# lzyhha/VisualCloze

Hardware: AMD Instinct MI355X
Metric: denoising-steps/sec (higher is better)
Workload: dtype bf16; 1 GPU; 384-grid-2x3 in-context, 30 solver points = 29 Flux evaluations per grid, L=512+3456 tokens, FLUX.1-Fill-dev geometry + LoRA r256 (merged), random-init weights, 1 independent grid(s) per GPU (data-parallel, no in-step collective); global_batch=1, seq_len=3968, parallelism=dp1

## Files before the change

### visualcloze_amd/csrc/attention64.hip

```cpp
#include <type_traits>
#include "common.h"
#include "vcloze_internal.h"
#include "attention64_sched8.h"

using namespace vcplan;

namespace {

struct Attn64Args {
  const bf16_t* qkv;
  const bf16_t* vt;
  bf16_t* out;
  const int32_t* kv_len;
  const int32_t* kv_gap;
  int64_t ld, bstride, ldo, out_bstride;
  int32_t B, L, Lpad, H, qblocks, items;
  int32_t full_rounds, tail_items, tail_units;
  float* part;
  const bf16_t* q_scale; const bf16_t* q_scale2; const float* rope; int64_t rope_bstride; int32_t split;
  int32_t q_pre;
  int32_t inmerge;
  uint32_t* flags;
  uint64_t* debug_ts;
};

constexpr int V_RING0 = RING * K_TILE;

constexpr int A_O = 0, A_Q = 128, A_K = 192;

typedef _Float16 f16x4 __attribute__((ext_vector_type(4)));
VC_DEV int chunk_begin64(int c, int units, int chunks) { return (int)(((long)c * units) / chunks); }
VC_DEV void merge_fold64(float (&acc)[16][4], float& wsum, float& m, const f16x4 (&v)[16], const f32x2 ml) {
  const float m_new = fmaxf(m, ml[0]);
  const float keep = __builtin_amdgcn_exp2f(m - m_new);
  const float w = ml[1] * __builtin_amdgcn_exp2f(ml[0] - m_new);
  m = m_new;
  wsum = __builtin_fmaf(wsum, keep, w);
#pragma unroll
  for (int i = 0; i < 16; ++i)
#pragma unroll
    for (int e = 0; e < 4; ++e) acc[i][e] = __builtin_fmaf(w, (float)v[i][e], acc[i][e] * keep);
}

VC_DEV int swap23(int i) { return (i & ~12) | ((i & 4) << 1) | ((i & 8) >> 1); }

template <int I, int N, class F>
VC_DEV void sfor(F&& f) {
  if constexpr (I < N) {
    f(std::integral_constant<int, I>{});
    sfor<I + 1, N>(f);
  }
}
#define SB() __builtin_amdgcn_sched_barrier(0)
template <int PH, int I>
constexpr a64s::Tok tok_at() {
  if constexpr (PH == 0) return a64s::A_TOK[I];
  else return a64s::B_TOK[I];
}

template <int KA, int QA, bool ZERO>
VC_DEV void mfma_qk(f32x16& s) {
  if constexpr (ZERO)
    asm volatile("v_mfma_f32_32x32x16_bf16 %0, a[%c1:%c2], a[%c3:%c4], 0" : "=v"(s) : "n"(KA), "n"(KA + 3), "n"(QA), "n"(QA + 3));
  else
    asm volatile("v_mfma_f32_32x32x16_bf16 %0, a[%c1:%c2], a[%c3:%c4], %0" : "+v"(s) : "n"(KA), "n"(KA + 3), "n"(QA), "n"(QA + 3));
}
VC_DEV void mfma_aug(f32x16& s, const u32x4& k, const u32x4& q) {
  asm volatile("v_mfma_f32_32x32x16_bf16 %0, %1, %2, %0" : "+v"(s) : "v"(k), "v"(q));
}
template <int OA>
VC_DEV void mfma_pv(const u32x4& v, const u32x4& p) {
  asm volatile("v_mfma_f32_32x32x16_bf16 a[%c2:%c3], %0, %1, a[%c2:%c3]" ::"v"(v), "v"(p), "n"(OA), "n"(OA + 15));
}
template <int A0, int OFF>
VC_DEV void lds_k(uint32_t addr) {
  asm volatile("ds_read_b128 a[%c1:%c2], %0 offset:%c3" ::"v"(addr), "n"(A0), "n"(A0 + 3), "n"(OFF));
}
template <int OFF>
VC_DEV void lds_v(u32x4& f, uint32_t addr) {
  asm volatile("ds_read_b128 %0, %1 offset:%c2" : "=v"(f) : "v"(addr), "n"(OFF));
}
template <int A0, int OFF>
VC_DEV void load_q(const bf16_t* p) {
  asm volatile("global_load_dwordx4 a[%c1:%c2], %0, off offset:%c3" ::"v"(p), "n"(A0), "n"(A0 + 3), "n"(OFF) : "memory");
}
template <int N> VC_DEV void wait_lgkm() { asm volatile("s_waitcnt lgkmcnt(%c0)" ::"n"(N)); }
template <int N> VC_DEV void wait_vm() { asm volatile("s_waitcnt vmcnt(%c0)" ::"n"(N)); }
VC_DEV float v_max3(float a, float b, float c) {
  float r;
  asm("v_max3_f32 %0, %1, %2, %3" : "=v"(r) : "v"(a), "v"(b), "v"(c));
  return r;
}
VC_DEV float v_max(float a, float b) {
  float r;
  asm("v_max_f32 %0, %1, %2" : "=v"(r) : "v"(a), "v"(b));
  return r;
}
#define PIN(x) asm volatile("" : "+v"(x))
VC_DEV uint32_t v_cvt_pk(float lo, float hi) {
  uint32_t r;
  asm("v_cvt_pk_bf16_f32 %0, %1, %2" : "=v"(r) : "v"(lo), "v"(hi));
  return r;
}
#pragma clang diagnostic push
#pragma clang diagnostic ignored "-Winline-asm"
VC_DEV void glds16_m0(const char* sbase, uint32_t voff, uint32_t lds_wave, int imm) {
  asm volatile("s_add_u32 m0, %2, %3\n\ts_nop 0\n\tglobal_load_lds_dwordx4 %0, %1" ::"v"(voff), "s"(sbase), "s"(lds_wave), "i"(imm) : "memory", "m0", "scc");
}
#pragma clang diagnostic pop
template <int A> VC_DEV float agpr_read() {
  float r;
  asm volatile("v_accvgpr_read_b32 %0, a[%c1]" : "=v"(r) : "n"(A));
  return r;
}
template <int A> VC_DEV void agpr_write(float v) { asm volatile("v_accvgpr_write_b32 a[%c1], %0" ::"v"(v), "n"(A)); }
VC_DEV void half_swap(float x, float& lo, float& hi) {
  asm volatile("v_mov_b32 %1, %2\n\tv_mov_b32 %0, %2\n\ts_nop 1\n\tv_permlane32_swap_b32 %0, %1" : "=&v"(lo), "=&v"(hi) : "v"(x));
}
VC_DEV float xmax32(float x) {
  float lo, hi;
  half_swap(x, lo, hi);
  return v_max(lo, hi);
}
VC_DEV float xsum32(float x) {
  float lo, hi;
  half_swap(x, lo, hi);
  return lo + hi;
}

template <bool BOUNDED>
__global__ __launch_bounds__(256, 1) void attn64_kernel(const Attn64Args a) {
  extern __shared__ __attribute__((aligned(16))) char smem[];
  asm volatile("" ::: "a0", "a15", "a31", "a47", "a63", "a79", "a95", "a111", "a127", "a143", "a159", "a175", "a191", "a207",
               "a223", "a239", "a255");

  const int tid = threadIdx.x;
  const int lane = tid & 63;
  const int wave = __builtin_amdgcn_readfirstlane(tid >> 6);
  const int lq = lane & 31, hh = lane >> 5;
  const float c_scale = 0.08838834764831845f * 1.4426950408889634f;
  const float MASKED = -29952.0f;

  uint32_t k_rd[8], v_rd[4];
  const int krow = swap23(lq);
  {
#pragma unroll
    for (int t = 0; t < 8; ++t) k_rd[t] = krow * 256 + (((2 * t + hh) ^ (krow & 15)) << 4);
#pragma unroll
    for (int s = 0; s < 4; ++s) v_rd[s] = V_RING0 + lq * 128 + (((2 * s + hh) ^ ((lq >> 1) & 7)) << 4);
  }
  uint32_t k_off[4], v_off[4];
#pragma unroll
  for (int i = 0; i < 4; ++i) {
    const int c = i * 256 + tid;
    const int row = c >> 4;
    k_off[i] = (uint32_t)row * (uint32_t)a.ld * 2u + (uint32_t)(((c & 15) ^ (row & 15)) << 4);
    const int d = c >> 3;
    v_off[i] = ((uint32_t)d * (uint32_t)a.Lpad + (uint32_t)((((c & 7) ^ ((d >> 1) & 7))) << 3)) * 2u;
  }
  const uint32_t k_step = (uint32_t)KVB * (uint32_t)a.ld * 2u;
  const uint32_t k_max = (uint32_t)(a.L - 1) * (uint32_t)a.ld * 2u + (uint32_t)(((tid & 15) ^ ((tid >> 4) & 15)) << 4);
  const uint32_t aug_on = hh == 0 ? 0xffffffffu : 0u;
  const uint32_t kaug_one = 0x3f80u & aug_on;
  const uint32_t qaug_mask = ((uint32_t)f2bf(MASKED) << 16) & aug_on;

#ifdef VC_ATTN_TIMESTAMPS
  const uint64_t ts0 = __builtin_amdgcn_s_memtime();
  int ts_tiles = 0, ts_seg = 0;
#define TS_SEG(k) do { if (a.debug_ts && tid == 0 && ts_seg < 3) a.debug_ts[blockIdx.x * 32 + 8 + ts_seg * 8 + (k)] = __builtin_amdgcn_s_memtime(); } while (0)
#else
#define TS_SEG(k) do { } while (0)
#endif
  const int G = gridDim.x;
  const int nkt_all = (a.L + KVB - 1) / KVB;
  const bool split = a.full_rounds >= 0;
  int tu = 0, tu_end = 0, it_first = 0, rounds_left = 0x7fffffff, id_full = blockIdx.x, id_step = G, id_tail = 0;
  if (split) {
    const int slot = blockIdx.x >> 3;
    const Sched64 sc = sched64(blockIdx.x & 7, G, a.items, nkt_all);
    tu = chunk_begin64(slot, sc.units, sc.W);
    tu_end = chunk_begin64(slot + 1, sc.units, sc.W);
    it_first = tu / nkt_all;
    rounds_left = sc.rounds;
    id_full = sc.start + slot;
    id_step = sc.W;
    id_tail = sc.start + sc.rounds * sc.W;
  }

  for (;;) {
    int id, kt0 = 0, kt1 = -1, piece = -1;
    if (rounds_left > 0) {
      if (!split && id_full >= a.items) break;
      id = split ? id_full : xcd_remap(id_full, a.items);
      id_full += id_step;
      --rounds_left;
    } else {
      if (tu >= tu_end) break;
      const int it = tu / nkt_all;
      kt0 = tu - it * nkt_all;
      kt1 = min(nkt_all, kt0 + (tu_end - tu));
      tu += kt1 - kt0;
      id = id_tail + it;
      if (kt1 - kt0 != nkt_all) piece = blockIdx.x * 2 + (it - it_first);
    }
    const int qb_i = id % a.qblocks;
    const int bh = id / a.qblocks;
    const int h = bh % a.H, b = bh / a.H;
    const int L = a.L;
    const int kvlen = a.kv_len ? __builtin_amdgcn_readfirstlane(a.kv_len[b]) : L;
    const int gap_lo = a.kv_gap ? __builtin_amdgcn_readfirstlane(a.kv_gap[2 * b]) : 0;
// ... 506 lines not shown
      id = id_tail + it;
      if (kt1 - kt0 != nkt_all) piece = blockIdx.x * 2 + (it - it_first);
    }
    const int bh = id / a.qblocks;
    const int h = bh % a.H, b = bh / a.H;
    n_id = id; n_kt0 = kt0; n_piece = piece;
    n_kvlen = a.kv_len ? __builtin_amdgcn_readfirstlane(a.kv_len[b]) : L;
    n_gap_lo = a.kv_gap ? __builtin_amdgcn_readfirstlane(a.kv_gap[2 * b]) : 0;
    n_gap_hi = a.kv_gap ? __builtin_amdgcn_readfirstlane(a.kv_gap[2 * b + 1]) : 0;
    n_kt1 = kt1 < 0 ? (n_kvlen + KVB - 1) / KVB : kt1;
    n_ko = ((uint32_t)b * (uint32_t)a.bstride + (uint32_t)(h * 128 + a.H * 128)) * 2u;
    n_vo = (uint32_t)(b * a.H + h) * 128u * (uint32_t)a.Lpad * 2u;
    return true;
  };
#define VC_SEG_ADVANCE do { c_id = n_id; c_kt0 = n_kt0; c_kt1 = n_kt1; c_piece = n_piece; c_kvlen = n_kvlen; c_gap_lo = n_gap_lo; \
                            c_gap_hi = n_gap_hi; c_ko = n_ko; c_vo = n_vo; have_next = next_seg(); } while (0)
  if (!next_seg()) return;
  VC_SEG_ADVANCE;

  using I0 = std::integral_constant<int, 0>;
  using I1 = std::integral_constant<int, 1>;
  using I2 = std::integral_constant<int, 2>;

  const uint32_t wave_lds = __builtin_amdgcn_readfirstlane((uint32_t)(uintptr_t)(lptr_t)(smem + wave * 1024));
  int pad1 = 0;
  auto src_tile = [&](int n, bool& fwd) __attribute__((always_inline)) -> int {
    fwd = n >= pad1 && have_next;
    return fwd ? min(n_kt0 + (n - pad1), n_kt1 - 1) : min(n, c_kt1 - 1);
  };
  const char* const k_base = (const char*)a.qkv;
  const char* const v_base = (const char*)a.vt;
  auto k_src = [&](int n, uint32_t& bound) __attribute__((always_inline)) -> uint32_t {
    bool fwd;
    const int kt = src_tile(n, fwd);
    const uint32_t so = fwd ? n_ko : c_ko;
    bound = k_bound + so;
    return (uint32_t)kt * k_step + so;
  };
  auto v_src = [&](int n) __attribute__((always_inline)) -> uint32_t {
    bool fwd;
    const int kt = src_tile(n, fwd);
    return (fwd ? n_vo : c_vo) + (uint32_t)kt * (KVB * 2);
  };
  auto dma_k_at = [&](auto SLOT, uint32_t sc, uint32_t bound, int i) __attribute__((always_inline)) {
#ifndef VC_A64_NO_DMA
    glds16_m0(k_base, min(k_off0 + (sc + (uint32_t)i * k_piece), bound), wave_lds, decltype(SLOT)::value * K_TILE + i * 4096);
#endif
  };
  auto dma_v_at = [&](auto SLOT, uint32_t sc, int i) __attribute__((always_inline)) {
#ifndef VC_A64_NO_DMA
    glds16_m0(v_base, v_off0 + (sc + (uint32_t)i * v_piece), wave_lds, V_RING0 + decltype(SLOT)::value * V_TILE + i * 4096);
#endif
  };
  auto dma_k = [&](auto SLOT, int n, int i) __attribute__((always_inline)) { uint32_t bd; const uint32_t sc = k_src(n, bd); dma_k_at(SLOT, sc, bd, i); };
  auto dma_v = [&](auto SLOT, int n, int i) __attribute__((always_inline)) { dma_v_at(SLOT, v_src(n), i); };
  auto load_queries = [&](int g_id) __attribute__((always_inline)) {
    const int qb_i = g_id % a.qblocks;
    const int bh = g_id / a.qblocks;
    const int h = bh % a.H, b = bh / a.H;
    const bf16_t* qbase = a.qkv + (long)b * a.bstride + h * 128;
    const int q0 = qb_i * QB + wave * QW;
    sfor<0, 2>([&](auto QBc) {
      constexpr int qb = decltype(QBc)::value;
      const int tok = min(q0 + qb * 32 + lq, L - 1);
      const bf16_t* qp = qbase + (long)tok * a.ld + hh * 8;
      sfor<0, 8>([&](auto T) { constexpr int t = decltype(T)::value; load_q<A_Q + (qb * 8 + t) * 4, t * 32>(qp); });
    });
  };

  f32x16 SBk[6];
  u32x4 P[2][4];
#pragma unroll
  for (int i = 0; i < 8; ++i) asm volatile("" : "=v"(P[i >> 2][i & 3]));
  u32x4 vf[a64s::V_REGS];
  u32x4 vfr[8];
#pragma unroll
  for (int i = 0; i < 8; ++i) asm volatile("" : "=v"(vfr[i]));
#pragma unroll
  for (int i = 0; i < a64s::V_REGS; ++i) asm volatile("" : "=v"(vf[i]));
  float l_acc[2] = {0.f, 0.f}, l_e[2] = {0.f, 0.f};
  float pe0[32], pe1[32];
  int pub = -1;
  bool dead = false;
#define VC_DEAD_OF(id) (BOUNDED && __builtin_amdgcn_readfirstlane((int)(((id) % a.qblocks) * QB + wave * QW >= L)) != 0)

  auto read_k = [&](auto SLOT, auto UT) __attribute__((always_inline)) {
    constexpr int ut = decltype(UT)::value, u = ut >> 3, t = ut & 7;
    lds_k<A_K + ut * 4, decltype(SLOT)::value * K_TILE + u * 8192>(k_rd[t]);
  };
  auto make_kaug = [&](int n, int u) __attribute__((always_inline)) -> u32x4 {
    const int key = n * KVB + u * 32 + krow;
    const uint32_t m = (key >= c_kvlen || (key >= c_gap_lo && key < c_gap_hi)) ? (0x3f800000u & aug_on) : 0u;
    return u32x4{kaug_one | m, 0u, 0u, 0u};
  };
  auto masked_step = [&](f32x16& Sx, int n, int u) __attribute__((always_inline)) {
    u32x4 ka = make_kaug(n, u);
    u32x4 qa = {qaug_mask, 0u, 0u, 0u};
    asm volatile("s_nop 7\n\tv_mfma_f32_32x32x16_bf16 %0, %1, %2, %0" : "+v"(Sx) : "v"(ka), "v"(qa));
  };
  auto tile_masked = [&](int n) __attribute__((always_inline)) { return n * KVB + KVB > c_kvlen || (n * KVB < c_gap_hi && n * KVB + KVB > c_gap_lo); };

  float m_run0 = 0.f, m_run1 = 0.f, alpha0 = 1.f, alpha1 = 1.f;
  u32x4 qaug_r0 = {qaug_mask, 0u, 0u, 0u}, qaug_r1 = {qaug_mask, 0u, 0u, 0u};
  int resc = 0;
  float mxp0 = 0.f, mxp1 = 0.f, mxp2 = 0.f, mxp3 = 0.f, mq0 = 0.f, mq1 = 0.f;
  auto max_step = [&](f32x16& Sx, float& mx, auto Jc) __attribute__((always_inline)) {
    constexpr int j = decltype(Jc)::value;
    if constexpr (j == 0) mx = v_max3(Sx[0], Sx[1], Sx[2]);
    else if constexpr (j < 7) mx = v_max3(mx, Sx[2 * j + 1], Sx[2 * j + 2]);
    else mx = v_max(mx, Sx[15]);
  };
  auto max_steps = [&](auto B0, auto Jc) __attribute__((always_inline)) {
    constexpr int b0 = decltype(B0)::value;
    max_step(SBk[(b0 + 0) % 6], mxp0, Jc);
    max_step(SBk[(b0 + 1) % 6], mxp1, Jc);
    max_step(SBk[(b0 + 2) % 6], mxp2, Jc);
    max_step(SBk[(b0 + 3) % 6], mxp3, Jc);
  };
  auto decide0 = [&]() __attribute__((always_inline)) {
    mq0 = v_max(mxp0, mxp1);
    mq1 = v_max(mxp2, mxp3);
  };
  auto decide1 = [&](auto QBc) __attribute__((always_inline)) { if constexpr (decltype(QBc)::value == 0) mq0 = xmax32(mq0); else mq1 = xmax32(mq1); };
  auto new_max = [&](float mq, float& m_run, float& alpha, u32x4& qa, f32x16& S0, f32x16& S1, bool first) __attribute__((always_inline)) {
    const float want = first ? mq : m_run + fmaxf(mq, 0.f);
    const bf16_t nb = f2bf(-want);
    const float m_new = -bf2f(nb);
    const float delta = m_new - m_run;
    alpha = __builtin_amdgcn_exp2f(-delta);
    m_run = m_new;
    qa[0] = ((uint32_t)nb & aug_on) | qaug_mask;
#pragma unroll
    for (int r = 0; r < 16; ++r) { S0[r] -= delta; S1[r] -= delta; }
  };
  auto decide2 = [&](auto B0, bool first) __attribute__((always_inline)) {
    constexpr int b0 = decltype(B0)::value;
    resc = (first || !__all((mq0 <= 8.0f) && (mq1 <= 8.0f))) ? 1 : 0;
    if (resc) {
      new_max(mq0, m_run0, alpha0, qaug_r0, SBk[(b0 + 0) % 6], SBk[(b0 + 1) % 6], first);
      new_max(mq1, m_run1, alpha1, qaug_r1, SBk[(b0 + 2) % 6], SBk[(b0 + 3) % 6], first);
    }
  };
  auto rescale_o = [&]() __attribute__((always_inline)) {
    if (resc) {
      asm volatile("s_nop 15\n\ts_nop 15" ::: "memory");
      sfor<0, 64>([&](auto I) { constexpr int i = decltype(I)::value; agpr_write<A_O + i>(agpr_read<A_O + i>() * alpha0); });
      sfor<64, 128>([&](auto I) { constexpr int i = decltype(I)::value; agpr_write<A_O + i>(agpr_read<A_O + i>() * alpha1); });
      l_acc[0] *= alpha0;
      l_acc[1] *= alpha1;
      asm volatile("s_nop 7" ::: "memory");
      resc = 0;
    }
  };
  auto tile_rs = [&](auto Jc, auto LASTc, int kt) __attribute__((always_inline)) {
    constexpr int J = decltype(Jc)::value;
    constexpr bool LAST = decltype(LASTc)::value, RK = !LAST || J == 1;
    constexpr int BASE = (4 * J) % 6;
    using SLOT_V = std::integral_constant<int, J>;
    using SLOT_K2 = std::integral_constant<int, (J + 2) % 3>;
    using SLOT_K4 = std::integral_constant<int, (J + 1) % 3>;
    rescale_o();
    const u32x4 ka0 = make_kaug(kt + 1, 0), ka1 = make_kaug(kt + 1, 1);
    uint32_t k_bd;
    uint32_t k_sc = k_src(kt + 4, k_bd), v_sc = v_src(kt + 2);
    VC_STREAM_PIN(k_sc, v_sc, k_bd);
    SB();
    float pe0r = 0.f, pe1r = 0.f;
    sfor<0, 36>([&](auto Gp) {
      constexpr int g = decltype(Gp)::value, c = g / 9, t = g % 9, qb = c >> 1, u = c & 1;
      if constexpr (!LAST) {
        if constexpr (t < 8) mfma_qk<A_K + (u * 8 + t) * 4, A_Q + (qb * 8 + t) * 4, t == 0>(SBk[(BASE + 4 + c) % 6]);
        else mfma_aug(SBk[(BASE + 4 + c) % 6], u == 0 ? ka0 : ka1, qb == 0 ? qaug_r0 : qaug_r1);
      }
      if constexpr (g > 0 && g <= 32) {
        constexpr int k = g - 1, pq = k >> 4, idx = k & 15, pu = idx >> 3, r0 = (idx & 7) * 2;
        l_acc[pq] += pe0r;
        l_acc[pq] += pe1r;
        PIN(l_acc[pq]);
        P[pq][pu * 2 + (r0 >> 3)][(r0 & 7) >> 1] = v_cvt_pk(pe0r, pe1r);
      }
      if constexpr (g < 32) {
        constexpr int k = g, pq = k >> 4, idx = k & 15, pu = idx >> 3, r0 = (idx & 7) * 2;
        pe0r = __builtin_amdgcn_exp2f(SBk[(BASE + pq * 2 + pu) % 6][r0]);
        pe1r = __builtin_amdgcn_exp2f(SBk[(BASE + pq * 2 + pu) % 6][r0 + 1]);
      }
      if constexpr (g >= 32) {
        constexpr int f = (g - 32) * 2;
        lds_v<SLOT_V::value * V_TILE + (f >> 2) * 4096>(vfr[f], v_rd[f & 3]);
        lds_v<SLOT_V::value * V_TILE + ((f + 1) >> 2) * 4096>(vfr[f + 1], v_rd[(f + 1) & 3]);
      }
      if constexpr (g == 35) wait_lgkm<0>();
      SB();
    });
    sfor<0, 32>([&](auto Gp) {
      constexpr int g = decltype(Gp)::value, dt = g >> 3, s = (g >> 1) & 3, qb = g & 1;
      if constexpr (g == 16) wait_lgkm<0>();
      mfma_pv<A_O + (qb * 4 + dt) * 16>(vfr[(dt & 1) * 4 + s], P[qb][s]);
      if constexpr (!LAST) {
        if constexpr (g >= 2 && g <= 9) max_steps(std::integral_constant<int, (BASE + 4) % 6>{}, std::integral_constant<int, g - 2>{});
        if constexpr (g == 10) decide0();
        if constexpr (g == 11) decide1(I0{});
        if constexpr (g == 12) decide1(I1{});
        if constexpr (g == 13) decide2(std::integral_constant<int, (BASE + 4) % 6>{}, false);
      }
      if constexpr ((g & 1) && g < 16) lds_v<SLOT_V::value * V_TILE + (dt + 2) * 4096>(vfr[(dt & 1) * 4 + s], v_rd[s]);
      if constexpr (RK && g >= 14 && g < 30) read_k(SLOT_K2{}, std::integral_constant<int, g - 14>{});
      if constexpr (g < 2 || (g >= 18 && g < 30 && (g & 1) == 0)) {
        constexpr int i = g < 2 ? g : (g - 18) / 2 + 2;
        if constexpr (i < 4) dma_v_at(SLOT_K2{}, v_sc, i);
        else dma_k_at(SLOT_K4{}, k_sc, k_bd, i - 4);
      }
      SB();
    });
    wait_vm<8>();
    wait_lgkm<0>();
    __builtin_amdgcn_s_barrier();
    SB();
  };
  auto run_tok = [&](auto PH, auto TI, auto LASTc, auto RKc, auto SBASE, auto SLOT_V, auto SLOT_K2, auto SLOT_K4, uint32_t v_sc, uint32_t k_sc, uint32_t k_bd) __attribute__((always_inline)) {
    constexpr a64s::Tok t = tok_at<decltype(PH)::value, decltype(TI)::value>();
    constexpr bool LAST = decltype(LASTc)::value, PB = decltype(PH)::value == 1, RK = decltype(RKc)::value;
    constexpr int k = t.a, pq = k >> 4, idx = k & 15, pu = idx >> 3, r0 = (idx & 7) * 2;
    constexpr int blk = (decltype(SBASE)::value + pq * 2 + pu) % 6;
    constexpr bool is_pair = t.kind <= a64s::T_CV;
#ifdef VC_A64_NO_SOFTMAX
    if constexpr (is_pair) return;
#endif
#ifdef VC_A64_NO_LDS
    if constexpr (t.kind == a64s::T_RV || t.kind == a64s::T_RV2 || t.kind == a64s::T_RK || t.kind == a64s::T_WAIT) return;
#endif
    if constexpr (is_pair && PB && LAST) { }
    else if constexpr (t.kind == a64s::T_E0) { pe0[k & 31] = __builtin_amdgcn_exp2f(SBk[blk][r0 & 15]); PIN(pe0[k & 31]); }
    else if constexpr (t.kind == a64s::T_E1) { pe1[k & 31] = __builtin_amdgcn_exp2f(SBk[blk][(r0 + 1) & 15]); PIN(pe1[k & 31]); }
    else if constexpr (t.kind == a64s::T_A0) {
      if constexpr (!PB) l_acc[pq & 1] += pe0[k & 31];
      else if constexpr (k != a64s::EARLY_FIRST[pq & 1]) l_e[pq & 1] += pe0[k & 31];
    } else if constexpr (t.kind == a64s::T_A1) {
      if constexpr (!PB) { l_acc[pq & 1] += pe1[k & 31]; PIN(l_acc[pq & 1]); }
      else if constexpr (k != a64s::EARLY_FIRST[pq & 1]) { l_e[pq & 1] += pe1[k & 31]; PIN(l_e[pq & 1]); }
      else { l_e[pq & 1] = pe0[k & 31] + pe1[k & 31]; PIN(l_e[pq & 1]); }
    }
    else if constexpr (t.kind == a64s::T_CV) P[pq & 1][(pu * 2 + (r0 >> 3)) & 3][(r0 & 7) >> 1] = v_cvt_pk(pe0[k & 31], pe1[k & 31]);
    else if constexpr (t.kind == a64s::T_RV)
      lds_v<decltype(SLOT_V)::value * V_TILE + (t.a & 3) * 4096>(vf[t.b % a64s::V_REGS], v_rd[(t.a >> 2) & 3]);
    else if constexpr (t.kind == a64s::T_RV2)
      lds_v<decltype(SLOT_V)::value * V_TILE + (t.a & 3) * 4096>(vf[t.b % a64s::V_REGS], v_rd[(t.a >> 2) & 3]);
    else if constexpr (t.kind == a64s::T_RK) { if constexpr (RK) read_k(SLOT_K2, std::integral_constant<int, t.a & 15>{}); }
    else if constexpr (t.kind == a64s::T_WAIT) { if constexpr (LAST) wait_lgkm<0>(); else wait_lgkm<t.a & 15>(); }
    else if constexpr (t.kind == a64s::T_DMA) {
      if constexpr (t.a < 4) dma_v_at(SLOT_K2, v_sc, t.a & 3);
      else dma_k_at(SLOT_K4, k_sc, k_bd, t.a & 3);
    }
  };
  auto tile_s = [&](auto Jc, auto LASTc, int kt) __attribute__((always_inline)) {
    constexpr int J = decltype(Jc)::value;
    constexpr bool LAST = decltype(LASTc)::value;
    using RKc = std::integral_constant<bool, !LAST || J == 1>;
    constexpr int BASE = (4 * J) % 6;
    using SLOT_V = std::integral_constant<int, J>;
    using SLOT_K2 = std::integral_constant<int, (J + 2) % 3>;
    using SLOT_K4 = std::integral_constant<int, (J + 1) % 3>;
    using SA = std::integral_constant<int, BASE>;
    using SB1 = std::integral_constant<int, (BASE + 4) % 6>;
    const bool msk = !LAST && tile_masked(kt + 1);
    uint32_t k_bd;
    uint32_t k_sc = k_src(kt + 4, k_bd), v_sc = v_src(kt + 2);
    VC_STREAM_PIN(k_sc, v_sc, k_bd);
    SB();
    sfor<0, 32>([&](auto Gp) {
      constexpr int g = decltype(Gp)::value, c = g >> 3, t = g & 7;
      if constexpr (!LAST) {
        mfma_qk<A_K + ((c & 1) * 8 + t) * 4, A_Q + ((c >> 1) * 8 + t) * 4, t == 0>(SBk[(BASE + 4 + c) % 6]);
        if constexpr (t == 7) { if (__builtin_expect(msk, 0)) masked_step(SBk[(BASE + 4 + c) % 6], kt + 1, c & 1); }
      }
      if constexpr (g == 0) {
        l_acc[0] += l_e[0];
        l_acc[1] += l_e[1];
      }
      sfor<a64s::A_FIRST[g], a64s::A_FIRST[g + 1]>([&](auto Ti) { run_tok(I0{}, Ti, LASTc, RKc{}, SA{}, SLOT_V{}, SLOT_K2{}, SLOT_K4{}, v_sc, k_sc, k_bd); });
      SB();
    });
    sfor<0, 32>([&](auto Gp) {
      constexpr int g = decltype(Gp)::value, s = g >> 3, dt = (g >> 1) & 3, qb = g & 1;
      mfma_pv<A_O + (qb * 4 + dt) * 16>(vf[a64s::PV_REG[g]], P[qb][s]);
      sfor<a64s::B_FIRST[g], a64s::B_FIRST[g + 1]>([&](auto Ti) { run_tok(I1{}, Ti, LASTc, RKc{}, SB1{}, SLOT_V{}, SLOT_K2{}, SLOT_K4{}, v_sc, k_sc, k_bd); });
      SB();
    });
#ifndef VC_A64_NO_DMA
    wait_vm<8>();
#endif
    wait_lgkm<0>();
#ifndef VC_A64_NO_BARRIER
    __builtin_amdgcn_s_barrier();
#endif
    SB();
  };
  auto dead_tile = [&](auto Jc, auto LASTc, int kt) __attribute__((always_inline)) {
    constexpr int J = decltype(Jc)::value;
    using SLOT_K2 = std::integral_constant<int, (J + 2) % 3>;
    using SLOT_K4 = std::integral_constant<int, (J + 1) % 3>;
    uint32_t k_bd;
    const uint32_t k_sc = k_src(kt + 4, k_bd), v_sc = v_src(kt + 2);
#pragma unroll
    for (int i = 0; i < 4; ++i) dma_v_at(SLOT_K2{}, v_sc, i);
    if (kt + 2 == pad1) sfor<0, 16>([&](auto UT) { read_k(SLOT_K2{}, UT); });
#pragma unroll
    for (int i = 0; i < 4; ++i) dma_k_at(SLOT_K4{}, k_sc, k_bd, i);
#ifndef VC_A64_NO_DMA
    wait_vm<8>();
#endif
    wait_lgkm<0>();
#ifndef VC_A64_NO_BARRIER
    __builtin_amdgcn_s_barrier();
#endif
    SB();
  };
  auto tile_any = [&](auto Jc, auto LASTc, int kt) __attribute__((always_inline)) {
    if constexpr (BOUNDED) tile_s(Jc, LASTc, kt);
    else tile_rs(Jc, LASTc, kt);
  };
  auto empty_s = [&](auto Jc, auto RKc, int n) __attribute__((always_inline)) {
    constexpr int J = decltype(Jc)::value;
    using SLOT_K2 = std::integral_constant<int, (J + 2) % 3>;
    using SLOT_K4 = std::integral_constant<int, (J + 1) % 3>;
#pragma unroll
    for (int i = 0; i < 4; ++i) dma_v(SLOT_K2{}, n + 2, i);
    if constexpr (decltype(RKc)::value) sfor<0, 16>([&](auto UT) { read_k(SLOT_K2{}, UT); });
#pragma unroll
    for (int i = 0; i < 4; ++i) dma_k(SLOT_K4{}, n + 4, i);
    wait_vm<8>();
    wait_lgkm<0>();
    __builtin_amdgcn_s_barrier();
    SB();
  };
  auto first_s = [&](bool hard_start) __attribute__((always_inline)) {
    const bool msk0 = tile_masked(c_kt0);
    SB();
    sfor<0, 32>([&](auto Gp) {
      constexpr int g = decltype(Gp)::value, c = g >> 3, t = g & 7;
      mfma_qk<A_K + ((c & 1) * 8 + t) * 4, A_Q + ((c >> 1) * 8 + t) * 4, t == 0>(SBk[c]);
      if constexpr (t == 7) {
        if (__builtin_expect(msk0, 0)) masked_step(SBk[c], c_kt0, c & 1);
      }
      sfor<0, 4>([&](auto Zc) { agpr_write<A_O + g * 4 + decltype(Zc)::value>(0.f); });
      SB();
    });
    if (hard_start) {
      wait_vm<16>();
      __builtin_amdgcn_s_barrier();
    }
    sfor<0, 16>([&](auto UT) { read_k(I1{}, UT); });
    asm volatile("s_nop 15" ::: "memory");
    SB();
    l_acc[0] = l_acc[1] = 0.f;
    l_e[0] = l_e[1] = 0.f;
    if constexpr (!BOUNDED) {
      m_run0 = m_run1 = 0.f;
      qaug_r0[0] = qaug_mask; qaug_r1[0] = qaug_mask;
      sfor<0, 8>([&](auto Jc) { max_steps(I0{}, Jc); });
      decide0();
      decide1(I0{});
      decide1(I1{});
      decide2(I0{}, true);
      resc = 0;
// ... 361 lines not shown
```

Measured before the change: 20.29 denoising-steps/sec.

## Drive attention tile loop from a table-generated interleaved instruction schedule

Replaces the hand-written interleaving of exp, row-sum, convert, V LDS reads, K reads, DMA issue and max/decide steps inside the flash-attention tile with a token table that spreads this work across the QK and PV MFMA slots. V reads are moved earlier into the QK phase, the max steps are spread over all PV slots, and the wait counts are relaxed. The aim is to hide VALU and LDS latency behind the MFMAs more evenly. It also keeps 32 exp results live in registers, which raises register pressure, and the hand-tuned wait counts are a correctness risk.

After: 20.28 denoising-steps/sec. No clear change (-0.0%).

```diff
diff --git a/visualcloze_amd/csrc/attention64.hip b/visualcloze_amd/csrc/attention64.hip
--- a/visualcloze_amd/csrc/attention64.hip
+++ b/visualcloze_amd/csrc/attention64.hip
@@ -2,6 +2,7 @@
 #include "common.h"
 #include "vcloze_internal.h"
 #include "attention64_sched8.h"
+#include "attention64_sched_rm.h"
 
 using namespace vcplan;
 
@@ -56,6 +57,11 @@
 constexpr a64s::Tok tok_at() {
   if constexpr (PH == 0) return a64s::A_TOK[I];
   else return a64s::B_TOK[I];
+}
+template <int PH, int I>
+constexpr a64r::Tok rtok_at() {
+  if constexpr (PH == 0) return a64r::A_TOK[I];
+  else return a64r::B_TOK[I];
 }
 
 template <int KA, int QA, bool ZERO>
@@ -868,64 +874,67 @@
       resc = 0;
     }
   };
+  auto run_tok_r = [&](auto PH, auto TI, auto LASTc, auto RKc, auto SBASE, auto SNEXT, auto SLOT_V, auto SLOT_K2, auto SLOT_K4, uint32_t v_sc, uint32_t k_sc, uint32_t k_bd) __attribute__((always_inline)) {
+    constexpr a64r::Tok t = rtok_at<decltype(PH)::value, decltype(TI)::value>();
+    constexpr bool LAST = decltype(LASTc)::value, RK = decltype(RKc)::value;
+    constexpr int k = t.a, pq = (k >> 4) & 1, idx = k & 15, pu = idx >> 3, r0 = (idx & 7) * 2;
+    constexpr int blk = (decltype(SBASE)::value + pq * 2 + pu) % 6;
+    constexpr int b1 = decltype(SNEXT)::value;
+    if constexpr (t.kind == a64r::T_E0) { pe0[k & 31] = __builtin_amdgcn_exp2f(SBk[blk][r0 & 15]); PIN(pe0[k & 31]); }
+    else if constexpr (t.kind == a64r::T_E1) { pe1[k & 31] = __builtin_amdgcn_exp2f(SBk[blk][(r0 + 1) & 15]); PIN(pe1[k & 31]); }
+    else if constexpr (t.kind == a64r::T_A0) l_acc[pq] += pe0[k & 31];
+    else if constexpr (t.kind == a64r::T_A1) { l_acc[pq] += pe1[k & 31]; PIN(l_acc[pq]); }
+    else if constexpr (t.kind == a64r::T_CV) P[pq][(pu * 2 + (r0 >> 3)) & 3][(r0 & 7) >> 1] = v_cvt_pk(pe0[k & 31], pe1[k & 31]);
+    else if constexpr (t.kind == a64r::T_RV || t.kind == a64r::T_RV2)
+      lds_v<decltype(SLOT_V)::value * V_TILE + (t.a & 3) * 4096>(vfr[t.b % a64r::V_REGS], v_rd[(t.a >> 2) & 3]);
+    else if constexpr (t.kind == a64r::T_RK) { if constexpr (RK) read_k(SLOT_K2, std::integral_constant<int, t.a & 15>{}); }
+    else if constexpr (t.kind == a64r::T_WAIT) { if constexpr (LAST) wait_lgkm<0>(); else wait_lgkm<t.a & 15>(); }
+    else if constexpr (t.kind == a64r::T_DMA) {
+      if constexpr (t.a < 4) dma_v_at(SLOT_K2, v_sc, t.a & 3);
+      else dma_k_at(SLOT_K4, k_sc, k_bd, t.a & 3);
+    }
+    else if constexpr (LAST) { }
+    else if constexpr (t.kind == a64r::T_MX) {
+      constexpr int c = (t.a >> 3) & 3;
+      using Jc = std::integral_constant<int, t.a & 7>;
+      if constexpr (c == 0) max_step(SBk[(b1 + 0) % 6], mxp0, Jc{});
+      else if constexpr (c == 1) max_step(SBk[(b1 + 1) % 6], mxp1, Jc{});
+      else if constexpr (c == 2) max_step(SBk[(b1 + 2) % 6], mxp2, Jc{});
+      else max_step(SBk[(b1 + 3) % 6], mxp3, Jc{});
+    }
+    else if constexpr (t.kind == a64r::T_D0) { if constexpr ((t.a & 1) == 0) mq0 = v_max(mxp0, mxp1); else mq1 = v_max(mxp2, mxp3); }
+    else if constexpr (t.kind == a64r::T_D1) decide1(std::integral_constant<int, t.a & 1>{});
+    else if constexpr (t.kind == a64r::T_D2) decide2(SNEXT, false);
+  };
   auto tile_rs = [&](auto Jc, auto LASTc, int kt) __attribute__((always_inline)) {
     constexpr int J = decltype(Jc)::value;
-    constexpr bool LAST = decltype(LASTc)::value, RK = !LAST || J == 1;
+    constexpr bool LAST = decltype(LASTc)::value;
+    using RKc = std::integral_constant<bool, !LAST || J == 1>;
     constexpr int BASE = (4 * J) % 6;
     using SLOT_V = std::integral_constant<int, J>;
     using SLOT_K2 = std::integral_constant<int, (J + 2) % 3>;
     using SLOT_K4 = std::integral_constant<int, (J + 1) % 3>;
+    using SA = std::integral_constant<int, BASE>;
+    using SB1 = std::integral_constant<int, (BASE + 4) % 6>;
     rescale_o();
     const u32x4 ka0 = make_kaug(kt + 1, 0), ka1 = make_kaug(kt + 1, 1);
     uint32_t k_bd;
     uint32_t k_sc = k_src(kt + 4, k_bd), v_sc = v_src(kt + 2);
     VC_STREAM_PIN(k_sc, v_sc, k_bd);
     SB();
-    float pe0r = 0.f, pe1r = 0.f;
     sfor<0, 36>([&](auto Gp) {
       constexpr int g = decltype(Gp)::value, c = g / 9, t = g % 9, qb = c >> 1, u = c & 1;
       if constexpr (!LAST) {
         if constexpr (t < 8) mfma_qk<A_K + (u * 8 + t) * 4, A_Q + (qb * 8 + t) * 4, t == 0>(SBk[(BASE + 4 + c) % 6]);
         else mfma_aug(SBk[(BASE + 4 + c) % 6], u == 0 ? ka0 : ka1, qb == 0 ? qaug_r0 : qaug_r1);
       }
-      if constexpr (g > 0 && g <= 32) {
-        constexpr int k = g - 1, pq = k >> 4, idx = k & 15, pu = idx >> 3, r0 = (idx & 7) * 2;
-        l_acc[pq] += pe0r;
-        l_acc[pq] += pe1r;
-        PIN(l_acc[pq]);
-        P[pq][pu * 2 + (r0 >> 3)][(r0 & 7) >> 1] = v_cvt_pk(pe0r, pe1r);
-      }
-      if constexpr (g < 32) {
-        constexpr int k = g, pq = k >> 4, idx = k & 15, pu = idx >> 3, r0 = (idx & 7) * 2;
-        pe0r = __builtin_amdgcn_exp2f(SBk[(BASE + pq * 2 + pu) % 6][r0]);
-        pe1r = __builtin_amdgcn_exp2f(SBk[(BASE + pq * 2 + pu) % 6][r0 + 1]);
-      }
-      if constexpr (g >= 32) {
-        constexpr int f = (g - 32) * 2;
-        lds_v<SLOT_V::value * V_TILE + (f >> 2) * 4096>(vfr[f], v_rd[f & 3]);
-        lds_v<SLOT_V::value * V_TILE + ((f + 1) >> 2) * 4096>(vfr[f + 1], v_rd[(f + 1) & 3]);
-      }
-      if constexpr (g == 35) wait_lgkm<0>();
+      sfor<a64r::A_FIRST[g], a64r::A_FIRST[g + 1]>([&](auto Ti) { run_tok_r(I0{}, Ti, LASTc, RKc{}, SA{}, SB1{}, SLOT_V{}, SLOT_K2{}, SLOT_K4{}, v_sc, k_sc, k_bd); });
       SB();
     });
     sfor<0, 32>([&](auto Gp) {
       constexpr int g = decltype(Gp)::value, dt = g >> 3, s = (g >> 1) & 3, qb = g & 1;
-      if constexpr (g == 16) wait_lgkm<0>();
-      mfma_pv<A_O + (qb * 4 + dt) * 16>(vfr[(dt & 1) * 4 + s], P[qb][s]);
-      if constexpr (!LAST) {
-        if constexpr (g >= 2 && g <= 9) max_steps(std::integral_constant<int, (BASE + 4) % 6>{}, std::integral_constant<int, g - 2>{});
-        if constexpr (g == 10) decide0();
-        if constexpr (g == 11) decide1(I0{});
-        if constexpr (g == 12) decide1(I1{});
-        if constexpr (g == 13) decide2(std::integral_constant<int, (BASE + 4) % 6>{}, false);
-      }
-      if constexpr ((g & 1) && g < 16) lds_v<SLOT_V::value * V_TILE + (dt + 2) * 4096>(vfr[(dt & 1) * 4 + s], v_rd[s]);
-      if constexpr (RK && g >= 14 && g < 30) read_k(SLOT_K2{}, std::integral_constant<int, g - 14>{});
-      if constexpr (g < 2 || (g >= 18 && g < 30 && (g & 1) == 0)) {
-        constexpr int i = g < 2 ? g : (g - 18) / 2 + 2;
-        if constexpr (i < 4) dma_v_at(SLOT_K2{}, v_sc, i);
-        else dma_k_at(SLOT_K4{}, k_sc, k_bd, i - 4);
-      }
+      mfma_pv<A_O + (qb * 4 + dt) * 16>(vfr[a64r::PV_REG[g]], P[qb][s]);
+      sfor<a64r::B_FIRST[g], a64r::B_FIRST[g + 1]>([&](auto Ti) { run_tok_r(I1{}, Ti, LASTc, RKc{}, SA{}, SB1{}, SLOT_V{}, SLOT_K2{}, SLOT_K4{}, v_sc, k_sc, k_bd); });
       SB();
     });
     wait_vm<8>();
diff --git a/visualcloze_amd/csrc/attention64_sched_rm.h b/visualcloze_amd/csrc/attention64_sched_rm.h
--- /dev/null
+++ b/visualcloze_amd/csrc/attention64_sched_rm.h
@@ -0,0 +1,11 @@
+#pragma once
+namespace a64r {
+enum : int { T_E0 = 0, T_E1 = 1, T_A0 = 2, T_A1 = 3, T_CV = 4, T_RV = 5, T_RV2 = 6, T_RK = 7, T_DMA = 8, T_WAIT = 9, T_MX = 10, T_D0 = 11, T_D1 = 12, T_D2 = 13 };
+struct Tok { int kind, a, b; };
+constexpr int V_REGS = 8;
+constexpr int PV_REG[32] = {0, 0, 1, 1, 2, 2, 3, 3, 4, 4, 5, 5, 6, 6, 7, 7, 0, 0, 1, 1, 2, 2, 3, 3, 4, 4, 5, 5, 6, 6, 7, 7};
+constexpr Tok A_TOK[169] = {{0, 0, 0}, {1, 0, 0}, {0, 1, 0}, {1, 1, 0}, {2, 0, 0}, {3, 0, 0}, {4, 0, 0}, {0, 2, 0}, {5, 0, 0}, {1, 2, 0}, {2, 1, 0}, {3, 1, 0}, {4, 1, 0}, {0, 3, 0}, {1, 3, 0}, {2, 2, 0}, {3, 2, 0}, {4, 2, 0}, {0, 4, 0}, {1, 4, 0}, {2, 3, 0}, {3, 3, 0}, {4, 3, 0}, {0, 5, 0}, {1, 5, 0}, {2, 4, 0}, {3, 4, 0}, {4, 4, 0}, {5, 4, 1}, {0, 6, 0}, {1, 6, 0}, {2, 5, 0}, {3, 5, 0}, {4, 5, 0}, {0, 7, 0}, {1, 7, 0}, {2, 6, 0}, {3, 6, 0}, {4, 6, 0}, {0, 8, 0}, {1, 8, 0}, {2, 7, 0}, {3, 7, 0}, {4, 7, 0}, {0, 9, 0}, {1, 9, 0}, {2, 8, 0}, {3, 8, 0}, {5, 8, 2}, {4, 8, 0}, {0, 10, 0}, {1, 10, 0}, {2, 9, 0}, {3, 9, 0}, {4, 9, 0}, {0, 11, 0}, {1, 11, 0}, {2, 10, 0}, {3, 10, 0}, {4, 10, 0}, {0, 12, 0}, {1, 12, 0}, {2, 11, 0}, {3, 11, 0}, {4, 11, 0}, {0, 13, 0}, {1, 13, 0}, {2, 12, 0}, {5, 12, 3}, {3, 12, 0}, {4, 12, 0}, {0, 14, 0}, {1, 14, 0}, {2, 13, 0}, {3, 13, 0}, {4, 13, 0}, {0, 15, 0}, {1, 15, 0}, {2, 14, 0}, {3, 14, 0}, {4, 14, 0}, {0, 16, 0}, {1, 16, 0}, {2, 15, 0}, {3, 15, 0}, {4, 15, 0}, {0, 17, 0}, {1, 17, 0}, {5, 1, 4}, {2, 16, 0}, {3, 16, 0}, {4, 16, 0}, {0, 18, 0}, {1, 18, 0}, {2, 17, 0}, {3, 17, 0}, {4, 17, 0}, {0, 19, 0}, {1, 19, 0}, {2, 18, 0}, {3, 18, 0}, {4, 18, 0}, {0, 20, 0}, {1, 20, 0}, {2, 19, 0}, {3, 19, 0}, {4, 19, 0}, {0, 21, 0}, {5, 5, 5}, {1, 21, 0}, {2, 20, 0}, {3, 20, 0}, {4, 20, 0}, {0, 22, 0}, {1, 22, 0}, {2, 21, 0}, {3, 21, 0}, {4, 21, 0}, {0, 23, 0}, {1, 23, 0}, {2, 22, 0}, {3, 22, 0}, {4, 22, 0}, {0, 24, 0}, {1, 24, 0}, {2, 23, 0}, {3, 23, 0}, {4, 23, 0}, {5, 9, 6}, {0, 25, 0}, {1, 25, 0}, {2, 24, 0}, {3, 24, 0}, {4, 24, 0}, {0, 26, 0}, {1, 26, 0}, {2, 25, 0}, {3, 25, 0}, {4, 25, 0}, {0, 27, 0}, {1, 27, 0}, {2, 26, 0}, {3, 26, 0}, {4, 26, 0}, {0, 28, 0}, {1, 28, 0}, {2, 27, 0}, {3, 27, 0}, {4, 27, 0}, {5, 13, 7}, {0, 29, 0}, {1, 29, 0}, {2, 28, 0}, {3, 28, 0}, {4, 28, 0}, {0, 30, 0}, {1, 30, 0}, {2, 29, 0}, {3, 29, 0}, {4, 29, 0}, {0, 31, 0}, {1, 31, 0}, {2, 30, 0}, {3, 30, 0}, {4, 30, 0}, {2, 31, 0}, {3, 31, 0}, {4, 31, 0}, {9, 4, 0}};
+constexpr int A_FIRST[37] = {0, 3, 8, 11, 16, 21, 26, 30, 35, 40, 45, 49, 53, 58, 63, 68, 72, 77, 82, 87, 91, 96, 101, 107, 110, 115, 120, 125, 129, 134, 139, 144, 149, 152, 157, 162, 169};
+constexpr Tok B_TOK[72] = {{10, 0, 0}, {8, 0, 0}, {10, 8, 0}, {6, 2, 0}, {10, 16, 0}, {10, 24, 0}, {7, 0, 0}, {10, 1, 0}, {6, 6, 1}, {10, 9, 0}, {10, 17, 0}, {7, 1, 0}, {8, 1, 0}, {10, 25, 0}, {10, 2, 0}, {6, 10, 2}, {10, 10, 0}, {7, 2, 0}, {9, 6, 0}, {10, 18, 0}, {10, 26, 0}, {6, 14, 3}, {10, 3, 0}, {10, 11, 0}, {7, 3, 0}, {8, 2, 0}, {10, 19, 0}, {6, 3, 4}, {10, 27, 0}, {10, 4, 0}, {7, 4, 0}, {10, 12, 0}, {10, 20, 0}, {6, 7, 5}, {10, 28, 0}, {7, 5, 0}, {10, 5, 0}, {8, 3, 0}, {9, 5, 0}, {10, 13, 0}, {6, 11, 6}, {10, 21, 0}, {7, 6, 0}, {10, 29, 0}, {10, 6, 0}, {6, 15, 7}, {10, 14, 0}, {7, 7, 0}, {10, 22, 0}, {8, 4, 0}, {10, 30, 0}, {10, 7, 0}, {7, 8, 0}, {10, 15, 0}, {10, 23, 0}, {10, 31, 0}, {7, 9, 0}, {11, 0, 0}, {11, 1, 0}, {8, 5, 0}, {9, 3, 0}, {7, 10, 0}, {12, 0, 0}, {7, 11, 0}, {12, 1, 0}, {8, 6, 0}, {7, 12, 0}, {7, 13, 0}, {13, 0, 0}, {8, 7, 0}, {7, 14, 0}, {7, 15, 0}};
+constexpr int B_FIRST[33] = {0, 2, 4, 7, 9, 12, 13, 16, 19, 22, 25, 26, 29, 32, 35, 37, 39, 41, 43, 46, 49, 50, 55, 59, 61, 62, 63, 65, 66, 68, 69, 70, 72};
+}
```
